# lammps/lammps-plugins

Hardware: AMD Instinct MI355X
Metric: Matom-steps/sec (higher is better)
Workload: dtype f64; 1 GPU; REBO-MoS bulk: in.rebomos-bulk cell replicated 24x24x24; atoms=3981312, style=rebomos, parallelism=spatial-dd1, transport=none (one GPU), rccl_library_is_test_double=False, thermo_every=10, displacement_check=every step, deferred on-device flag, dangerous_builds=0, inner_skin=adaptive from 1.0, late_style_list_builds_rank0=0, row_prunings_late_rank0=0, rccl_ranks=1

## Files before the change

include/mdpair_hip.h:

```cpp
#ifndef MDPAIR_HIP_H
#define MDPAIR_HIP_H

#include <stddef.h>
#include <stdint.h>

#ifdef __cplusplus
extern "C" {
#endif

#define MDP_ABI_VERSION 3

enum {
  MDP_OK = 0,
  MDP_EINVAL = -1,
  MDP_EHIP = -2,
  MDP_ENOMEM = -3,
  MDP_EOVERFLOW = -4,
  MDP_ENOTIMPL = -5,
  MDP_ESTATE = -6
};

#define MDP_EFLAG_GLOBAL 1
#define MDP_EFLAG_ATOM 2
#define MDP_VFLAG_GLOBAL 1
// ... 85 lines not shown
} mdp_md_config;

int mdp_md_setup(mdp_ctx *ctx, const mdp_md_config *cfg, const double *x, const double *v, const int *type,
                 const int *tag, const double *mass, const int *map, const int *ghost_owner,
                 const double *ghost_shift, const int *ghost_type, const int *ghost_tag);
int mdp_md_build_neighbors(mdp_ctx *ctx);
int mdp_md_initial_integrate(mdp_ctx *ctx);
int mdp_md_final_integrate(mdp_ctx *ctx);
int mdp_md_final_initial_integrate(mdp_ctx *ctx);
int mdp_md_defer_final(mdp_ctx *ctx);
int mdp_md_compute(mdp_ctx *ctx, int eflag, int vflag);
int mdp_md_compute_begin(mdp_ctx *ctx, int eflag, int vflag);
int mdp_md_compute_end(mdp_ctx *ctx, int eflag, int vflag);
int mdp_md_pack_x(mdp_ctx *ctx, int n, const int *d_sendlist, const double *d_shift, double *d_buf);
int mdp_md_unpack_x(mdp_ctx *ctx, int first_ghost, int n, const double *d_buf);
int mdp_md_pack_scalar(mdp_ctx *ctx, int which, int n, const int *d_sendlist, double *d_buf);
int mdp_md_unpack_scalar(mdp_ctx *ctx, int which, int first_ghost, int n, const double *d_buf);
int mdp_md_pack_ghost_f(mdp_ctx *ctx, int first_ghost, int n, double *d_buf);
int mdp_md_unpack_add_f(mdp_ctx *ctx, int n, const int *d_sendlist, const double *d_buf);
int mdp_md_fold_self_ghost_f(mdp_ctx *ctx);
int mdp_md_aeam_density(mdp_ctx *ctx, int eflag);
int mdp_md_aeam_force_begin(mdp_ctx *ctx, int eflag, int vflag);
int mdp_md_aeam_force(mdp_ctx *ctx, int eflag, int vflag);
int mdp_md_aeam_state(mdp_ctx *ctx, int out[4]);
int mdp_md_thermo(mdp_ctx *ctx, double out[9]);
int mdp_md_download(mdp_ctx *ctx, double *x, double *v, double *f, double *eatom);
int mdp_md_upload_x(mdp_ctx *ctx, const double *x);
int mdp_md_download_x_all(mdp_ctx *ctx, double *x_all);
void *mdp_md_ptr(mdp_ctx *ctx, const char *name);
int mdp_md_neighbor_stats(mdp_ctx *ctx, long long out[8]);
int mdp_md_prune_stats(mdp_ctx *ctx, long long out[4]);
int mdp_md_list_state(mdp_ctx *ctx, double out[8]);
int mdp_rebomos_list_info(mdp_ctx *ctx, long long out[8]);
int mdp_md_class_stats(mdp_ctx *ctx, long long out[32]);

typedef struct {
  double boxlo[3];
  double h[6];
  int procgrid[3];
  int rank;
  double cutghost;
  int self_remote;
  int nonperiodic[3];
} mdp_dd_config;

int mdp_dd_setup(mdp_ctx *ctx, const mdp_dd_config *cfg);
int mdp_dd_reneighbor(mdp_ctx *ctx);
int mdp_dd_migrate_begin(mdp_ctx *ctx, int *send_counts );
int mdp_dd_migrate_pack(mdp_ctx *ctx, double *d_buf);
int mdp_dd_migrate_end(mdp_ctx *ctx, int narrive, const double *d_buf);
int mdp_dd_borders_begin(mdp_ctx *ctx, int *send_counts );
int mdp_dd_borders_pack(mdp_ctx *ctx, double *d_buf);
int mdp_dd_borders_end(mdp_ctx *ctx, const int *recv_counts , const double *d_buf);
int mdp_dd_info(mdp_ctx *ctx, long long out[8], int *send_counts, int *recv_counts);
int mdp_dd_forward_pack(mdp_ctx *ctx, double *d_buf);
int mdp_dd_forward_unpack(mdp_ctx *ctx, const double *d_buf);
int mdp_dd_forward_scalar_pack(mdp_ctx *ctx, double *d_buf);
int mdp_dd_forward_scalar_unpack(mdp_ctx *ctx, const double *d_buf);
int mdp_dd_reverse_pack(mdp_ctx *ctx, double *d_buf);
int mdp_dd_reverse_unpack(mdp_ctx *ctx, const double *d_buf);
int mdp_dd_comm_unique_id(void *id128);
int mdp_dd_comm_library(char *buf, int cap);
int mdp_dd_comm_init(mdp_ctx *ctx, const void *id128);
int mdp_dd_comm_destroy(mdp_ctx *ctx);
int mdp_dd_comm_reneighbor(mdp_ctx *ctx);
int mdp_dd_comm_forward_begin(mdp_ctx *ctx);
// ... 94 lines not shown
```

lammps-plugins_amd/csrc/md.hip:

```cpp
#include "mdp_common.h"

#include <rocprim/rocprim.hpp>

#include <cmath>
#include <type_traits>

void mdp_rebomos_fill_dev(mdp_ctx *c, double skin);

namespace {

struct CutTables {
  double owned[MDP_AEAM_MAXT * MDP_AEAM_MAXT];
  double ghost[MDP_AEAM_MAXT * MDP_AEAM_MAXT];
  const double *g_owned;
  int ne;
  int min_type;
};

using Grid = MdpGrid;

__device__ __forceinline__ int cell_index(const Grid &g, const double4 &x, int &cx, int &cy, int &cz)
{
  cx = (int) ((x.x - g.lo[0]) * g.inv[0]);
  cy = (int) ((x.y - g.lo[1]) * g.inv[1]);
// ... 1538 lines not shown
  CutTables ct;
  memset(&ct, 0, sizeof ct);
  double maxcut = 0.0;
  MDP_TRY(aeam_cut_table(c, ct, skin, maxcut));
  return host_list_compare(c, ct, maxcut, host_total, "aeam");
}

void *mdp_md_ptr(mdp_ctx *c, const char *name)
{
  if (!c || !name) return nullptr;
  if (!strcmp(name, "x")) return c->xq.p;
  if (!strcmp(name, "v")) return c->v.p;
  if (!strcmp(name, "f")) return c->f.p;
  if (!strcmp(name, "fp")) return c->fp.p;
  if (!strcmp(name, "eatom")) return c->eatom.p;
  return nullptr;
}

int mdp_rebomos_list_info(mdp_ctx *c, long long out[8])
{
  if (!c || !out) return MDP_EINVAL;
  if (!c->rebo_packed) return mdp_fail(c, MDP_ESTATE, "rebomos lists not built yet");
  out[0] = c->lj_tiled ? 1 : 0;
  out[1] = c->ntile;
  out[2] = c->tile_cap;
  out[3] = c->tile_maxu;
  out[4] = c->lj_total;
  out[5] = c->nclus;
  out[6] = (c->lj_class_base[2] - c->lj_class_base[1]) + (c->lj_class_base[4] - c->lj_class_base[3]);
  out[7] = c->style_builds;
  return MDP_OK;
}

int mdp_md_class_stats(mdp_ctx *c, long long out[32])
{
  if (!c || !out) return MDP_EINVAL;
  for (int k = 0; k < 32; k++) out[k] = 0;
  out[30] = c->tile_maxu;
  if (c->cfg.style == 2 || (c->have_aeam && !c->have_rebomos)) {
    out[0] = c->h_ang_count;
    out[1] = c->ntile;
    out[2] = c->aeam_split;
    return MDP_OK;
  }
  for (int k = 0; k < MDP_NCLASS; k++) out[k] = c->h_class_count[k];
  for (int k = 0; k < 4; k++) out[20 + k] = c->lj_class_base[k + 1] - c->lj_class_base[k];
  if (c->lj_tiled && !c->lj_ordered) out[20] = c->ntile;
  if (c->h_pinned) {
    const int *h = mdp_pin(c, kPinOvf) + 4 * c->ovf_par;
    for (int k = 0; k < 4; k++) out[25 + k] = h[k];
    out[24] = *mdp_pin(c, kPinGeneral);
  }
  out[29] = c->tile_small;
  return MDP_OK;
}

int mdp_md_neighbor_stats(mdp_ctx *c, long long out[8])
{
  if (!c || !out) return MDP_EINVAL;
  for (int k = 0; k < 8; k++) out[k] = 0;
  out[0] = c->nb_owned_total;
  out[1] = c->nb_total - c->nb_owned_total;
  out[2] = c->lj_total;
  out[3] = c->cand_total;
  out[4] = 0;
  for (int k = 0; k < MDP_NCLASS; k++) out[4] += c->h_class_count[k];
// ... 110 lines not shown
```

lammps-plugins_amd/csrc/mdp_api.hip:

```cpp
#include "mdp_common.h"

#include <rocprim/rocprim.hpp>

#include <condition_variable>
#include <functional>
#include <mutex>
#include <thread>
#include <unistd.h>

#include <cmath>

void mdp_rebomos_fill_dev(mdp_ctx *c, double skin);

int mdp_fail(mdp_ctx *c, int code, const char *fmt, ...)
{
  char buf[1024];
  va_list ap;
  va_start(ap, fmt);
  vsnprintf(buf, sizeof buf, fmt, ap);
  va_end(ap);
  if (c) c->err = buf;
  return code;
}

// ... 731 lines not shown
  c->vatom.release();
  c->acc.release();
  c->flags.release();
  c->nb_off.release();
  c->nb.release();
  c->cand_cnt.release();
  c->cand_off.release();
  c->cand.release();
  c->lj_off.release();
  c->lj_cnt.release();
  c->lj_split.release();
  c->cl_flag.release();
  c->cl_pos.release();
  c->cl_order.release();
  c->lj.release();
  c->tu.release();
  c->tmask.release();
  c->lj16_in.release();
  c->lj_len_in.release();
  c->lj_split_in.release();
  c->cand_stage.release();
  c->lj_fixtab.release();
  c->lj_fix_stamp.release();
  c->xhold_prune.release();
  c->tile_nu.release();
  c->tile_flag.release();
  c->lj16.release();
  c->is_center.release();
  c->class_list.release();
  c->class_merged.release();
  c->class_count.release();
  c->pk_cand.release();
  c->amask.release();
  c->xhold_all.release();
  c->ovf.release();
  c->rev.release();
  c->rev16.release();
  c->host_perm.release();
  c->host_tagmap.release();
  c->host_inv.release();
  c->host_tag_dev.release();
  c->host_img.release();
  c->host_stage.release();
  host_unregister_all(c);
  for (int k = 0; k < MDP_DOWN_CHUNKS; k++)
    if (c->ev_down[k]) {
      (void) hipEventDestroy(c->ev_down[k]);
      c->ev_down[k] = nullptr;
    }
  for (int k = 0; k < MDP_UP_RING; k++) {
    if (c->h_up[k]) (void) hipHostFree(c->h_up[k]);
    if (c->ev_up[k]) (void) hipEventDestroy(c->ev_up[k]);
    c->h_up[k] = nullptr;
    c->ev_up[k] = nullptr;
  }
  if (c->h_down) (void) hipHostFree(c->h_down);
  c->h_down = nullptr;
  c->fnbr.release();
  c->fown.release();
  c->vslot.release();
  c->scan_tmp.release();
  c->rho.release();
  c->fp.release();
  c->ang_list.release();
  c->ang_count.release();
  c->v.release();
// ... 470 lines not shown
```

lammps-plugins_amd/csrc/mdp_common.h:

```cpp
#pragma once

#include <hip/hip_runtime.h>

#include <atomic>
#include <cstdarg>
#include <cstdio>
#include <cstdlib>
#include <cstring>
#include <string>
#include <utility>
#include <vector>

#include "mdpair_hip.h"

#define MDP_NEIGHMASK 0x1FFFFFFF
#define MDP_CLUSTER 2
static_assert(MDP_CLUSTER == 1 || MDP_CLUSTER == 2, "the Lennard-Jones kernels are instantiated for 1- and 2-atom clusters only");
#define MDP_ACC_SLOTS 512
#define MDP_ACC_STRIDE 16
#define MDP_NOVF_LISTS 7
#define MDP_NCLASS 20
#define MDP_NCLASS_HALF 10

inline std::atomic<long long> &mdp_device_bytes_counter()
// ... 504 lines not shown
  DevBuf<unsigned short> lj16;
  DevBuf<int> is_center;
  bool hn_on = false;
  double hn_dt = 0.0, hn_dtf = 0.0, hn_ftm2v = 0.0;
  double hn_mass[16] = {};
  DevBuf<double> hn_mass_dev;
  bool hn_v_current = false;
  int ovf_par = 0;
  bool hn_deferred_check = false;
  int ang_list_n = -1;
  bool f_prezeroed = false;
  bool f_zero_remote_due = false;
  bool aeam_img_fp = false;
  DevBuf<int> lj_fix_stamp;
  int lj_stamp = 0;
  DevBuf<unsigned short> lj_cq;
  DevBuf<int> lj_cq_cnt;
  int lj_cq_cap = 0, lj_cq_tiles = 0;
  bool lj_queue_now = false;
  DevBuf<double> lj_fixtab;
  DevBuf<int> cand_stage;
  DevBuf<int> class_list;
  DevBuf<int> class_count;
  DevBuf<int> pk_cand;
  size_t pk_base[MDP_NCLASS] = {};
  DevBuf<int> class_merged;
  size_t merged_base[MDP_NCLASS_HALF] = {};
  int h_class_count[MDP_NCLASS] = {};
  DevBuf<unsigned long long> amask;
  DevBuf<int> rev;
  DevBuf<int> rev16;
  DevBuf<int> ovf;
  int ovf_stride = 0;
  int ovf3_hot[4] = {0, 0, 0, 0};
  DevBuf<mdp_hold_t> xhold_all;
  double skin_inner = 0.0;
  double skin_inner_auto = 1.0;
  double skin_inner_cap = 1.0e9;
  long long computes_since_build = 0;
  bool stale_rebuild = false;
  long long style_builds = 0;
  long long dangerous_builds = 0;
  int sflag_set = 0;
  bool sflag_armed = false;
  bool sflag_committed[2] = {false, false};
  MdpStyleCheck sflag_chk;
  MdpStyleCheckMeta sflag_meta[2];
  hipEvent_t ev_sflag[2] = {nullptr, nullptr};
  MdpNhc nhc;
  MdpLangevin lgv;
  MdpFire fire;
  DevBuf<int> mask;
  bool mask_set = false;
  int mask_n = 0;
  int group_bit = 0, lgv_bit = 0;
  DevBuf<int> image;
  bool image_set = false;
  MdpMsd msd;
  MdpRdf rdf;
  bool final_pending = false;
  bool final_deferred_seen = false;
  bool acc_prezeroed = false;
  bool check_now = false;
  DevBuf<double> fnbr;
  DevBuf<double> fown;
  DevBuf<double> vslot;
// ... 158 lines not shown
```

lammps-plugins_amd/csrc/rebomos.hip:

```cpp
#include "mdp_common.h"

#include <type_traits>

namespace {

#ifndef MDP_LJ_WAVES
#define MDP_LJ_WAVES 4
#endif
constexpr double kPi = 3.14159265358979323846;
constexpr double kTol = 1.0e-9;

__device__ __forceinline__ void wave_lds_fence()
{
  __builtin_amdgcn_fence(__ATOMIC_RELEASE, "wavefront");
  __builtin_amdgcn_wave_barrier();
  __builtin_amdgcn_fence(__ATOMIC_ACQUIRE, "wavefront");
}

template <int G> __device__ __forceinline__ double group_sum_any(double v, const int s, const int lane);

__device__ __forceinline__ int xcd_contiguous(const int b, const int n)
{
  const int q = n >> 3, r = n & 7, xcd = b & 7, idx = b >> 3;
  return xcd * q + (xcd < r ? xcd : r) + idx;
}

template <int G> __device__ __forceinline__ double group_sum_any(double v, const int s, const int lane)
{
  if constexpr ((G & (G - 1)) == 0) {
    return group_sum<G>(v);
  } else {
    static_assert(G <= 16, "tree below starts at offset 8");
#pragma unroll
    for (int o = 8; o > 0; o >>= 1) {
      const double t = __shfl_down(v, o, 64);
// ... 18 lines not shown
  double y = __builtin_amdgcn_rcp(x);
  double e = fma(-x, y, 1.0);
  y = fma(y, e, y);
  e = fma(-x, y, 1.0);
  return fma(y, e, y);
}

__device__ __forceinline__ double rsqrt_nr(double x)
{
  double y = __builtin_amdgcn_rsq(x);
  double e = fma(-x * y, y, 1.0);
  y = fma(0.5 * y, e, y);
  e = fma(-x * y, y, 1.0);
  return fma(0.5 * y, e, y);
}

__device__ __forceinline__ double sp_switch(double r, double rmin, double rinv, double &dw)
{
  const double t = (r - rmin) * rinv;
  if (t <= 0.0) {
    dw = 0.0;
    return 1.0;
  }
  if (t >= 1.0) {
    dw = 0.0;
    return 0.0;
  }
  double s, c;
  sincospi(t, &s, &c);
  dw = -0.5 * kPi * s * rinv;
  return 0.5 * (1.0 + c);
}

__device__ __forceinline__ void sincospi_half(const double u, double &sn, double &cs)
{
  const bool fold = u > 0.25;
  const double v = fold ? 0.5 - u : u;
  const double w = v * v;
  constexpr double S[8] = {3.14159265358979312e+00, -5.16771278004996937e+00, 2.55016403987734508e+00, -5.99264529320791883e-01, 8.21458866111281910e-02, -7.37043094571434784e-03, 4.66302805767612337e-04, -2.19153534478302037e-05};
  constexpr double C[9] = {1.00000000000000000e+00, -4.93480220054467900e+00, 4.05871212641676760e+00, -1.33526276885458928e+00, 2.35330630358893123e-01, -2.58068913900140508e-02, 1.92957430940392206e-03, -1.04638104924845650e-04, 4.30306958703294391e-06};
  double ps = S[7], pc = C[8];
#pragma unroll
  for (int k = 6; k >= 0; k--) ps = fma(ps, w, S[k]);
#pragma unroll
  for (int k = 7; k >= 0; k--) pc = fma(pc, w, C[k]);
  ps *= v;
  sn = fold ? pc : ps;
  cs = fold ? ps : pc;
}

__device__ __forceinline__ double poly6(const double *c, double x, double &d)
{
  double g = c[6] * x, dg = 6.0 * c[6] * x;
  g += c[5];
  dg += 5.0 * c[5];
  g *= x;
  dg *= x;
  g += c[4];
  dg += 4.0 * c[4];
  g *= x;
  dg *= x;
  g += c[3];
  dg += 3.0 * c[3];
  g *= x;
  dg *= x;
  g += c[2];
  dg += 2.0 * c[2];
  g *= x;
  dg *= x;
  g += c[1];
  dg += c[1];
  g *= x;
  g += c[0];
  d = dg;
  return g;
}

__device__ __forceinline__ double poly6v(const double *c, double x)
{
  return (((((c[6] * x + c[5]) * x + c[4]) * x + c[3]) * x + c[2]) * x + c[1]) * x + c[0];
}

__device__ __forceinline__ double gspline_val(const double *cb, const double *cg, double c)
{
  const double gcos = poly6v(cb, c);
  if (c < 0.5) return gcos;
  const double gamma = poly6v(cg, c);
  const double psi = 0.5 * (1.0 - cospi(2.0 * (c - 0.5)));
  return gcos + psi * (gamma - gcos);
}

__device__ __forceinline__ double gspline(const double *cb, const double *cg, double c, double &dgdc)
{
  if (c < 0.5) {
    return poly6(cb, c, dgdc);
  }
  double dgcos, dgamma;
  const double gcos = poly6(cb, c, dgcos);
  const double gamma = poly6(cg, c, dgamma);
  double s, co;
  sincospi_half(c - 0.5, s, co);
  const double psi = s * s;
  const double dpsi = 2.0 * kPi * s * co;
  dgdc = dgcos + dpsi * (gamma - gcos) + psi * (dgamma - dgcos);
  return gcos + psi * (gamma - gcos);
}

constexpr int kRec = 10;
constexpr int kRecF = 9, kInvF = 7;

struct CentreOut {
  double e_acc, v0, v1, v2, v3, v4, v5;
};

__device__ __forceinline__ void finish_slot(const RebomosDev &P, const int tc, const int je_m, const int off,
                                            const double dp, const bool owned, const int eflag, const double mx,
                                            const double my, const double mz, const double mr, const double mw,
                                            const double mdw, const double mp, const double mrinv, const double mVA,
                                            double &fx, double &fy, double &fz, const double acc1, const double Csum,
                                            double *__restrict__ fnbr, double &eh, CentreOut &o)
{
  const int tm = ((unsigned) je_m) >> 30;
  const int pt = tc * 2 + tm;
  const double ux = mx * mrinv, uy = my * mrinv, uz = mz * mrinv;
  double radial = (acc1 + Csum * dp) * mdw;
  double ehalf = 0.0;
  if (mw > kTol) {
    const double ex = exp(-P.alpha[pt] * mr);
    const double pre = mw * P.A[pt] * ex;
    const double VR = pre * (1.0 + P.Q[pt] * mrinv);
    double dVR = pre * (-P.alpha[pt] - P.Q[pt] * mrinv * mrinv - P.Q[pt] * P.alpha[pt] * mrinv);
    const double swl = fast_rcp(mw) * mdw;
    dVR += VR * swl;
    double dVA = -P.beta[pt] * mVA;
    dVA += mVA * swl;
    radial += 0.5 * (dVR + mp * dVA);
    ehalf = 0.5 * (VR + mp * mVA);
  }
// ... 49 lines not shown
  const double rsq = dx * dx + dy * dy + dz * dz;
  const int tj = (int) xj.w;
  const double rc2 = P.rcmaxsq[tc * 2 + tj];
  const bool pred = valid && rsq < rc2;
  if (valid && !pred && rsq < rc2 * (1.0 + 1.0e-14)) {
    slot4[t] = make_double4(0.0, 0.0, 0.0, 0.0);
    if (vslot)
      for (int k = 0; k < 6; k++) vslot[6 * (size_t) t + k] = 0.0;
  }
  const unsigned long long bal = __ballot(pred);
  const unsigned long long gb = (bal >> glane0) & gmask;
  const int pos = n + __popcll(gb & ((1ull << s) - 1ull));
  if (pred && pos < CAP) {
    const int pt = tc * 2 + tj;
    const double rinv = rsqrt_nr(rsq);
    const double r = rsq * rinv;
    double dw;
    const double w = sp_switch(r, P.rcmin[pt], P.rcinv[pt], dw);
    double *q = rec + pos * REC;
    q[0] = dx;
    q[1] = dy;
    q[2] = dz;
    q[3] = r;
    q[4] = w;
    q[5] = dw;
    q[REC == kRec ? 8 : kInvF] = rinv;
    je[pos] = t | (tj << 30);
    nsum += w;
  }
  n += __popcll(gb);
  if (base < 64) active |= gb << base;
}

template <int G> struct CentreCfg {
  static constexpr int CAP = G;
  static constexpr int GPW = 64 / G;
  static constexpr int WPB = G == 12 ? 3 : 4;
  static constexpr int STRIDE = CAP * kRecF + 2;
  static constexpr int MSTRIDE = 2 * (G / 2) * G + 2;
  static constexpr int UA = G >= 32 ? 1 : (G >= 12 ? 2 : 4);
};


template <int G, bool LIST = false>
__global__ __launch_bounds__(64 * CentreCfg<G>::WPB) void rebo_centre_kernel(
    const RebomosDev P, const int *__restrict__ centres, const int ncent_arg, const int nlocal,
    const double4 *__restrict__ xq, const int *__restrict__ cand_off, const int *__restrict__ cand,
    const int *__restrict__ pk, unsigned long long *__restrict__ amask, double *__restrict__ fnbr,
    double *__restrict__ fown, double *__restrict__ acc, int *__restrict__ ovf, const int eflag, const int vflag,
    const int tc )
{
  using C = CentreCfg<G>;
  __shared__ double s_rec[C::WPB * C::GPW * C::STRIDE];
  __shared__ double s_mat[C::WPB * C::GPW * C::MSTRIDE];
  __shared__ int s_je[C::WPB * C::GPW * C::CAP];

  const int tid = threadIdx.x;
  const int lane = tid & 63;
  const int s = lane % G;
  const int glane0 = lane - s;
  const int gw = lane / G;
  const bool lane_ok = gw < C::GPW;
  const int grp_in_block = (tid >> 6) * C::GPW + (lane_ok ? gw : C::GPW - 1);
  const long long gid = (long long) (LIST ? (int) blockIdx.x : xcd_contiguous(blockIdx.x, gridDim.x)) * (C::WPB * C::GPW) + grp_in_block;
  const int ncent = LIST ? centres[-1] : ncent_arg;
  const bool have = lane_ok && gid < ncent;
  if (LIST) {
    int *h_count = reinterpret_cast<int *>(const_cast<int *>(pk));
    if (blockIdx.x == 0 && tid == 0) *h_count = ncent;
    const long long covered = (long long) gridDim.x * (C::WPB * C::GPW);
    for (long long e = covered + (long long) blockIdx.x * blockDim.x + tid; e < ncent; e += (long long) gridDim.x * blockDim.x)
      ovf[1 + atomicAdd(&ovf[0], 1)] = centres[e];
  }

  double *rec = s_rec + (size_t) grp_in_block * C::STRIDE;
  double *mat = s_mat + (size_t) grp_in_block * C::MSTRIDE;
  int *je = s_je + grp_in_block * C::CAP;

  constexpr int W = C::UA * G;
  int jp[C::UA];
  if (!LIST) {
#pragma unroll
    for (int u = 0; u < C::UA; u++) jp[u] = have ? pk[(size_t) gid * W + u * G + s] : -1;
// ... 17 lines not shown
  {
    double4 xj[C::UA];
#pragma unroll
    for (int u = 0; u < C::UA; u++) xj[u] = xq[jp[u] >= 0 ? jp[u] : c];
#pragma unroll
    for (int u = 0; u < C::UA; u++)
      centre_take<G, C::CAP, kRecF>(P, tc, xc, jp[u] >= 0, u * G + s, xj[u], s, glane0, u * G, rec, je, n, active, nsum,
                                    reinterpret_cast<double4 *>(fnbr) + off, nullptr);
  }
  const int ncw = wave_max_int(nc);
  for (int base = W; base < ncw; base += W) {
    int jj[C::UA];
    double4 xj[C::UA];
#pragma unroll
    for (int u = 0; u < C::UA; u++) {
      const int t = base + u * G + s;
      jj[u] = t < nc ? cand[off + t] : c;
    }
#pragma unroll
    for (int u = 0; u < C::UA; u++) xj[u] = xq[jj[u]];
#pragma unroll
    for (int u = 0; u < C::UA; u++) {
      const int t = base + u * G + s;
      centre_take<G, C::CAP, kRecF>(P, tc, xc, t < nc, t, xj[u], s, glane0, base + u * G, rec, je, n, active, nsum,
                                    reinterpret_cast<double4 *>(fnbr) + off, nullptr);
    }
  }
  if (have && s == 0) amask[c] = active;
  const bool outgrown = n > C::CAP;
  if (outgrown) {
    if (s == 0) ovf[1 + atomicAdd(&ovf[0], 1)] = c;
    n = 0;
  }
  const double Ntot = group_sum_any<G>(nsum, s, lane);
  wave_lds_fence();

  double cb[7], cg[7];
#pragma unroll
  for (int k = 0; k < 7; k++) {
    cb[k] = P.b[tc][k];
    cg[k] = P.bg[tc][k];
  }
  const double ea = exp(-P.a[tc][2] * Ntot);
  const double dp = -P.a[tc][0] + P.a[tc][1] * P.a[tc][2] * ea;
  const double PS = -P.a[tc][0] * (Ntot - 1.0) - P.a[tc][1] * ea + P.a[tc][3];

  const int nw = wave_max_int(n);
  CentreOut o = {0, 0, 0, 0, 0, 0, 0};
  const bool owned = have && c < nlocal;

  const int m = s;
  const bool act = m < n;
  double mx = 0, my = 0, mz = 0, mr = 1, mw = 0, mdw = 0, mri = 1;
  if (act) {
    const double *q = rec + m * kRecF;
    mx = q[0];
    my = q[1];
    mz = q[2];
    mr = q[3];
    mw = q[4];
    mdw = q[5];
    mri = q[kInvF];
  }
  const double ux = mx * mri, uy = my * mri, uz = mz * mri;
  const int lane_base = (threadIdx.x & 63) - s;
  double S = 0.0;
  for (int d = 1; d <= nw / 2; d++) {
    const bool mine = act && (2 * d < n || (2 * d == n && m < d));
    double give = 0.0;
    if (mine) {
      int qi = m + d;
      qi = qi >= n ? qi - n : qi;
      const double *q = rec + qi * kRecF;
      double cs = (ux * q[0] + uy * q[1] + uz * q[2]) * q[kInvF];
      cs = fmin(cs, 1.0);
      cs = fmax(cs, -1.0);
      double dg, g;
      if (__any(cs >= 0.5)) g = gspline(cb, cg, cs, dg);
      else g = poly6(cb, cs, dg);
      double *e = mat + 2 * ((d - 1) * G + m);
      e[0] = g;
      e[1] = dg;
      S += q[4] * g;
      give = mw * g;
    }
    int src = m - d;
    src = src < 0 ? src + n : src;
    const double got = __shfl(give, lane_base + (act ? src : m), 64);
    S += act ? got : 0.0;
  }
  double mC = 0.0, mp = 0.0, mVA = 0.0;
  if (act) {
    const int pt = tc * 2 + (((unsigned) je[m]) >> 30);
    mp = rsqrt_nr(1.0 + S + PS);
    mVA = -mw * P.B[pt] * exp(-P.beta[pt] * mr);
    mC = (mw > kTol) ? 0.5 * mVA * (-0.5 * mp * mp * mp) : 0.0;
    rec[m * kRecF + 6] = mC;
  }
  const double Csum = group_sum_any<G>(mC, s, lane);
  wave_lds_fence();
  double fx = 0, fy = 0, fz = 0, acc1 = 0;
  for (int d = 1; d <= nw / 2; d++) {
    const bool mine = act && (2 * d < n || (2 * d == n && m < d));
    double sx = 0, sy = 0, sz = 0, sa = 0;
    if (mine) {
      int qi = m + d;
      qi = qi >= n ? qi - n : qi;
      const double *q = rec + qi * kRecF;
      const double qrinv = q[kInvF];
      const double qx = q[0] * qrinv, qy = q[1] * qrinv, qz = q[2] * qrinv;
      double cs = ux * qx + uy * qy + uz * qz;
      cs = fmin(cs, 1.0);
      cs = fmax(cs, -1.0);
      const double *e = mat + 2 * ((d - 1) * G + m);
      const double g = e[0], dg = e[1];
      const double common = (mC * q[4] + q[6] * mw) * dg;
      const double cm = common * mri, cq = common * qrinv;
      fx += cm * (qx - cs * ux);
      fy += cm * (qy - cs * uy);
      fz += cm * (qz - cs * uz);
      acc1 += q[6] * g;
      sx = cq * (ux - cs * qx);
      sy = cq * (uy - cs * qy);
      sz = cq * (uz - cs * qz);
      sa = mC * g;
    }
    int src = m - d;
    src = src < 0 ? src + n : src;
    const int from = lane_base + (act ? src : m);
    const double rx = __shfl(sx, from, 64), ry = __shfl(sy, from, 64), rz = __shfl(sz, from, 64);
    const double ra = __shfl(sa, from, 64);
    if (act) {
      fx += rx;
      fy += ry;
      fz += rz;
      acc1 += ra;
    }
  }
  double eh = 0.0;
  if (act)
    finish_slot(P, tc, je[m], off, dp, owned, eflag, mx, my, mz, mr, mw, mdw, mp, mri, mVA, fx, fy, fz, acc1, Csum,
                fnbr, eh, o);
  const double ox = group_sum_any<G>(act ? fx : 0.0, s, lane), oy = group_sum_any<G>(act ? fy : 0.0, s, lane), oz = group_sum_any<G>(act ? fz : 0.0, s, lane);
  const double oe = (eflag & MDP_EFLAG_ATOM) ? group_sum_any<G>(eh, s, lane) : 0.0;
  if (owned && s == 0 && !outgrown) reinterpret_cast<double4 *>(fown)[c] = make_double4(-ox, -oy, -oz, oe);
  centre_tally(o, acc, eflag, vflag);
}

constexpr int kC3Block = 256;
__global__ __launch_bounds__(kC3Block) void rebo_centre3_kernel(
    const RebomosDev P, const int *__restrict__ centres, const int ncent, const int nlocal,
    const double4 *__restrict__ xq, const int *__restrict__ cand_off, const int *__restrict__ cand,
    const int *__restrict__ pk, unsigned long long *__restrict__ amask, double *__restrict__ fnbr,
    double *__restrict__ fown, double *__restrict__ acc, int *__restrict__ ovf3 ,
    int *__restrict__ ovf_general , const int eflag, const int vflag, const int tc)
{
  constexpr int W = CentreCfg<4>::UA * 4;
  static_assert(W == 16, "four int4 per centre");
  const long long gid = (long long) xcd_contiguous(blockIdx.x, gridDim.x) * kC3Block + threadIdx.x;
  const bool have = gid < ncent;
  int jp[W];
  {
    const int4 *__restrict__ p4 = reinterpret_cast<const int4 *>(pk) + (have ? gid : 0) * (W / 4);
#pragma unroll
    for (int q = 0; q < W / 4; q++) {
      const int4 v = p4[q];
      jp[4 * q] = have ? v.x : -1;
      jp[4 * q + 1] = have ? v.y : -1;
      jp[4 * q + 2] = have ? v.z : -1;
      jp[4 * q + 3] = have ? v.w : -1;
    }
  }
  int c = 0, off = 0, nc = 0;
  double4 xc = make_double4(0, 0, 0, 0);
  if (have) {
    c = centres[gid];
    off = cand_off[c];
    nc = cand_off[c + 1] - off;
// ... 2897 lines not shown
  if (c->md || !c->have_rebomos || c->have_aeam || !c->rebo_packed || !c->nall) return MDP_OK;
  MDP_TRY(rebomos_check_launch(c, 0.5 * c->skin_inner));
  c->host_check_armed = true;
  return MDP_OK;
}

static int rebomos_lists_stale(mdp_ctx *c, bool &stale)
{
  stale = false;
  if (!c->nall) return MDP_OK;
  int *h = mdp_pin(c, kPinHostCheck);
  if (!c->md && c->host_check_armed) {
    c->host_check_armed = false;
    stale = h[0] != 0;
    if (c->prune_valid && h[2]) c->prune_stale = true;
    return MDP_OK;
  }
  const bool deferred_host = !c->md && c->hn_on && c->hn_deferred_check && !c->check_now;
  if ((!c->md && !deferred_host) || c->check_now) {
    mdp_sflag_drop(c);
    c->check_now = false;
    MDP_TRY(rebomos_check_launch(c, 0.5 * c->skin_inner));
    MDP_HIP(c, hipStreamSynchronize(c->stream));
    stale = h[0] != 0;
    if (c->prune_valid && h[2]) c->prune_stale = true;
    return MDP_OK;
  }
  bool toofar = false;
  MDP_TRY(mdp_sflag_collect(c, &stale, &toofar));
  if (toofar) c->dangerous_builds++;
  return MDP_OK;
}

template <int G>
static void launch_centre(mdp_ctx *c, int kg, int eflag, int vflag, int part)
{
  for (int elem = 0; elem < 2; elem++) {
    const int k = 2 * kg + elem + (part == 1 ? MDP_NCLASS_HALF : 0);
    const int n = c->h_class_count[k] + (part == 2 ? c->h_class_count[k + MDP_NCLASS_HALF] : 0);
    if (n <= 0) continue;
    const int *list = part == 2 ? c->class_merged.p + c->merged_base[k] : c->class_list.p + (size_t) k * c->nall;
    constexpr int per_block = CentreCfg<G>::WPB * CentreCfg<G>::GPW;
    const int grid = (n + per_block - 1) / per_block;
    rebo_centre_kernel<G><<<grid, 64 * CentreCfg<G>::WPB, 0, c->stream>>>(c->rebomos, list, n, c->nlocal,
                                                       c->xq.p, c->cand_off.p, c->cand.p, c->pk_cand.p + c->pk_base[k],
                                                       c->amask.p, c->fnbr.p, c->fown.p, c->acc.p, c->ovf.p, eflag, vflag,
                                                       elem);
  }
}

static void launch_centre3(mdp_ctx *c, int eflag, int vflag, int part)
{
  for (int elem = 0; elem < 2; elem++) {
    const int k = elem + (part == 1 ? MDP_NCLASS_HALF : 0);
    const int n = c->h_class_count[k] + (part == 2 ? c->h_class_count[k + MDP_NCLASS_HALF] : 0);
    if (n <= 0) continue;
    const int *clist = part == 2 ? c->class_merged.p + c->merged_base[k] : c->class_list.p + (size_t) k * c->nall;
    const int q = (part == 1 ? 2 : 0) + elem;
    int *list = c->ovf.p + (size_t) (q + 1) * c->ovf_stride + 1;
    int *h_cnt = mdp_pin(c, kPinOvf) + 4 * c->ovf_par + q;
    if (*h_cnt > 0) c->ovf3_hot[q] = 64;
    else if (c->ovf3_hot[q] > 0) c->ovf3_hot[q]--;
    const bool list_mode = c->ovf3_hot[q] > 0;
    rebo_centre3_kernel<<<(n + kC3Block - 1) / kC3Block, kC3Block, 0, c->stream>>>(c->rebomos, clist, n,
                                                                c->nlocal, c->xq.p, c->cand_off.p, c->cand.p,
                                                                c->pk_cand.p + c->pk_base[k], c->amask.p, c->fnbr.p,
                                                                c->fown.p, c->acc.p, list, list_mode ? nullptr : c->ovf.p,
                                                                eflag, vflag, elem);
    if (!list_mode) continue;
    constexpr int per_block = CentreCfg<8>::WPB * CentreCfg<8>::GPW;
    long long est = 4 * (long long) *h_cnt + 2 * per_block;
    if (est > n) est = n;
    const int grid = (int) ((est + per_block - 1) / per_block);
    rebo_centre_kernel<8, true><<<grid, 64 * CentreCfg<8>::WPB, 0, c->stream>>>(
        c->rebomos, list, 0, c->nlocal, c->xq.p, c->cand_off.p, c->cand.p, h_cnt, c->amask.p, c->fnbr.p, c->fown.p,
        c->acc.p, c->ovf.p, eflag, vflag, elem);
  }
}

int mdp_tile_prune(mdp_ctx *c, const double lim_rsq[4])
{
  hipStream_t st = c->stream;
  const int nrow = c->ntile * MDP_TILE;
  MDP_HIP(c, c->lj_len_in.reserve(nrow + 1));
  MDP_HIP(c, c->lj_split_in.reserve(nrow + 1));
  MDP_HIP(c, c->xhold_prune.reserve((size_t) 3 * c->nall + 3));
  if (c->prune_copied_epoch != c->prune_epoch) {
    MDP_HIP(c, c->lj16_in.reserve((size_t) c->lj_total + 256));
    MDP_HIP(c, hipMemcpyAsync(c->lj16_in.p + c->lj_total, c->lj16.p + c->lj_total, sizeof(unsigned short) * 256,
                              hipMemcpyDeviceToDevice, st));
    c->prune_copied_epoch = c->prune_epoch;
  }
  PruneLimits lim;
  for (int k = 0; k < 4; k++) lim.rsq[k] = lim_rsq[k];
  const int capL = (c->tile_maxu + 1 + 1) & ~1;
  const size_t lds = (size_t) capL * 3 * sizeof(double) + (size_t) 2 * c->tile_rowmax + 32;
  if (c->tile_rowmax <= 0 || lds > 160 * 1024) {
    c->prune_valid = false;
    return MDP_OK;
  }
#define MDP_TP(CLV)                                                                                                    \
  do {                                                                                                                 \
    if (lds > 48 * 1024)                                                                                               \
      MDP_HIP(c, hipFuncSetAttribute((const void *) tile_prune_kernel<CLV>, hipFuncAttributeMaxDynamicSharedMemorySize, \
                                     (int) lds));                                                                      \
    tile_prune_kernel<CLV><<<c->ntile, 256, lds, st>>>(lim, c->nlocal, c->nclus, c->xq.p, c->tile_cap, capL, c->tu.p,    \
                                                       c->tile_nu.p, c->lj_off.p, c->lj_split.p, c->lj16.p,            \
                                                       c->lj16_in.p, c->lj_len_in.p, c->lj_split_in.p);               \
  } while (0)
// ... 172 lines not shown
    MDP_HIP(c, hipGetLastError());
  }
  const int capL = (c->tile_maxu + 1 + 7) & ~7;
  const size_t lds = (size_t) capL * 3 * sizeof(double);
  int *h_count = mdp_pin(c, queue ? kPinCubicWalk : kPinCubic);
  long long want = (long long) *h_count + *h_count / 4 + 256;
  const int grid = (int) (want < c->ntile ? want : c->ntile);
  const int *fix_list = c->ovf.p + (size_t) (queue ? 6 : 5) * c->ovf_stride;
#define MDP_LJC(CLV, EVV)                                                                                            \
  do {                                                                                                                \
    if (lds > 48 * 1024)                                                                                              \
      MDP_HIP(c, hipFuncSetAttribute((const void *) rebo_lj_cubic_kernel<CLV, EVV>,                                   \
                                     hipFuncAttributeMaxDynamicSharedMemorySize, (int) lds));                         \
    rebo_lj_cubic_kernel<CLV, EVV><<<grid, 256, lds, c->stream>>>(                                                    \
        c->lj_fixtab.p, fix_list, c->nlocal, c->nclus, c->xq.p, c->tile_cap, c->tu.p, c->tile_nu.p, c->lj_off.p,      \
        pruned ? c->lj_len_in.p : nullptr, pruned ? c->lj_split_in.p : c->lj_split.p,                                 \
        pruned ? c->lj16_in.p : c->lj16.p, c->f.p, c->eatom.p, c->acc.p, eflag, vflag, h_count);                      \
  } while (0)
  const bool ev = eflag || vflag;
  if (c->cluster == 1) {
    if (ev) MDP_LJC(1, true);
    else MDP_LJC(1, false);
  } else {
    if (ev) MDP_LJC(2, true);
    else MDP_LJC(2, false);
  }
#undef MDP_LJC
  MDP_HIP(c, hipGetLastError());
  return MDP_OK;
}

static int launch_centres(mdp_ctx *c, int eflag, int vflag, int parts, int which = 3, bool first = true)
{
  if ((parts & 1) && first) c->ovf_par ^= 1;
  hipStream_t st = c->stream;
  if (c->centre_split && parts == 3 && which == 3) {
    launch_centre3(c, eflag, vflag, 2);
    launch_centre<8>(c, 1, eflag, vflag, 2);
    launch_centre<12>(c, 2, eflag, vflag, 2);
    launch_centre<16>(c, 3, eflag, vflag, 2);
    launch_centre<32>(c, 4, eflag, vflag, 2);
  } else
    for (int part = 0; part < 2; part++) {
      if (!((parts >> part) & 1)) continue;
      const int w = part == 0 ? which : 3;
      if (w & 1) launch_centre3(c, eflag, vflag, part);
      if (w & 2) {
        launch_centre<8>(c, 1, eflag, vflag, part);
        launch_centre<12>(c, 2, eflag, vflag, part);
        launch_centre<16>(c, 3, eflag, vflag, part);
        launch_centre<32>(c, 4, eflag, vflag, part);
      }
    }
  MDP_HIP(c, hipGetLastError());
  if (!(parts & 2)) return MDP_OK;
  int total = 0;
  for (int k = 0; k < MDP_NCLASS; k++) total += c->h_class_count[k];
  const int grid = total > 0 ? (total / 8 + 1 < 64 ? total / 8 + 1 : 64) : 0;
  mdp_time_mark(c, 1);
  if (grid)
    rebo_centre_general_kernel<false><<<grid, 256, 0, st>>>(c->rebomos, c->ovf.p, -1, c->nlocal, c->xq.p,
                                                            c->cand_off.p, c->cand.p, c->amask.p, c->fnbr.p,
                                                            c->fown.p, nullptr, nullptr, c->acc.p, c->flags.p,
                                                            eflag, vflag, mdp_pin(c, kPinOvf) + 4 * c->ovf_par,
                                                            c->ovf_stride, mdp_pin(c, kPinGeneral));
  MDP_HIP(c, hipGetLastError());
// ... 114 lines not shown
```

lammps-plugins_amd/host/capi.py:

```python
from __future__ import annotations

import ctypes as C
import os

import numpy as np

PKG_DIR = os.path.dirname(os.path.dirname(os.path.abspath(__file__)))
LIB_PATH = os.path.join(PKG_DIR, "libmdpair_hip.so")

D22 = (C.c_double * 2) * 2


class RebomosParams(C.Structure):
    _fields_ = [(n, D22) for n in ("rcmin", "rcmax", "rcmaxsq", "Q", "alpha", "A", "BIJc", "Beta")] + [
        ("b", (C.c_double * 2) * 7), ("bg", (C.c_double * 2) * 7), ("a", (C.c_double * 2) * 4)] + [
        (n, D22) for n in ("rcLJmin", "rcLJmax", "epsilon", "sigma", "lj1", "lj2", "lj3", "lj4")]


class AeamTables(C.Structure):
    _fields_ = [("ntypes", C.c_int), ("nelements", C.c_int), ("nnonangular", C.c_int),
                ("nrhomax", C.c_int), ("nrmax", C.c_int), ("nfrho", C.c_int), ("nrhor", C.c_int), ("nz2r", C.c_int),
                ("nrho", C.POINTER(C.c_int)), ("drho", C.POINTER(C.c_double)),
                ("nr", C.POINTER(C.c_int)), ("dr", C.POINTER(C.c_double)), ("cut", C.POINTER(C.c_double)),
                ("type2frho", C.POINTER(C.c_int)), ("type2rhor", C.POINTER(C.c_int)), ("type2z2r", C.POINTER(C.c_int)),
# ... 36 lines not shown
FIRE_DEFAULTS = dict(dmax=0.1, tmax=10.0, tmin=0.02, delaystep=20, dtgrow=1.1, dtshrink=0.5, alpha0=0.25,
                     alphashrink=0.99, halfstepback=True, initialdelay=True)
BOLTZ_METAL = 8.617343e-5


STYLE_REBOMOS, STYLE_AEAM = 1, 2
EXPORTS = [
    "mdp_abi_version", "mdp_device_count", "mdp_create", "mdp_destroy", "mdp_last_error", "mdp_set_stream",
    "mdp_sync", "mdp_rebomos_set_params", "mdp_rebomos_read_file", "mdp_rebomos_params_from_scalars",
    "mdp_aeam_set_tables", "mdp_aeam_file_read", "mdp_aeam_file_info", "mdp_aeam_file_build", "mdp_aeam_file_free", "mdp_set_atoms_host", "mdp_set_positions_host",
    "mdp_set_box_host", "mdp_host_ghosts_derived",
    "mdp_set_neighbors_host", "mdp_set_skin", "mdp_set_neighbors_csr_host", "mdp_rebomos_compute_host", "mdp_aeam_density_host",
    "mdp_aeam_force_host", "mdp_md_setup", "mdp_md_build_neighbors", "mdp_md_initial_integrate",
    "mdp_md_final_integrate", "mdp_md_final_initial_integrate", "mdp_md_compute", "mdp_md_compute_begin", "mdp_md_compute_end", "mdp_md_pack_x", "mdp_md_unpack_x", "mdp_md_pack_scalar",
    "mdp_md_unpack_scalar", "mdp_md_pack_ghost_f", "mdp_md_unpack_add_f", "mdp_md_fold_self_ghost_f",
    "mdp_md_aeam_density", "mdp_md_aeam_force", "mdp_md_thermo", "mdp_md_download", "mdp_md_upload_x", "mdp_md_ptr",
    "mdp_md_neighbor_stats", "mdp_md_class_stats", "mdp_md_prune_stats", "mdp_hnve_setup", "mdp_hnve_off", "mdp_hnve_upload_v",
    "mdp_hnve_initial", "mdp_hnve_final", "mdp_hnve_download", "mdp_rebomos_list_info", "mdp_set_timing", "mdp_get_timing",
    "mdp_device_bytes", "mdp_host_release", "mdp_rebomos_check_host_list",
    "mdp_dd_setup", "mdp_dd_reneighbor", "mdp_dd_migrate_begin", "mdp_dd_migrate_pack", "mdp_dd_migrate_end",
    "mdp_dd_borders_begin", "mdp_dd_borders_pack", "mdp_dd_borders_end", "mdp_dd_info", "mdp_dd_forward_pack",
    "mdp_dd_forward_unpack", "mdp_dd_forward_scalar_pack", "mdp_dd_forward_scalar_unpack", "mdp_dd_reverse_pack",
    "mdp_dd_reverse_unpack", "mdp_md_moved_async", "mdp_md_integrate_check", "mdp_md_download_int", "mdp_md_download_x_all",
    "mdp_dd_comm_unique_id", "mdp_dd_comm_library", "mdp_dd_comm_init", "mdp_dd_comm_destroy", "mdp_dd_comm_reneighbor",
    "mdp_dd_comm_forward_begin", "mdp_dd_comm_forward_end", "mdp_dd_comm_forward_scalar", "mdp_dd_comm_reverse",
    "mdp_dd_comm_allreduce", "mdp_dd_comm_step_begin", "mdp_dd_comm_step_end", "mdp_dd_comm_step_info", "mdp_aeam_device_lists", "mdp_rebomos_host_list", "mdp_aeam_check_host_list",
    "mdp_md_defer_final", "mdp_md_list_state", "mdp_md_aeam_force_begin", "mdp_md_aeam_state", "mdp_dd_comm_aeam_exchange_begin", "mdp_dd_comm_aeam_exchange_end",
    "mdp_nhc_setup", "mdp_nhc_run", "mdp_nhc_state", "mdp_nhc_set_state", "mdp_nhc_off",
    "mdp_langevin_setup", "mdp_langevin_run", "mdp_langevin_tally", "mdp_langevin_off",
    "mdp_fire_setup", "mdp_fire_iterate", "mdp_fire_state", "mdp_fire_off",
    "mdp_md_set_mask", "mdp_hnve_set_mask", "mdp_integrate_group", "mdp_langevin_group",
    "mdp_md_set_image", "mdp_md_download_unwrapped", "mdp_msd_setup", "mdp_msd_sums", "mdp_msd_info", "mdp_msd_off",
    "mdp_rdf_setup", "mdp_rdf_counts", "mdp_rdf_info", "mdp_rdf_off",
]


class MdpError(RuntimeError):
    def __init__(self, code, text):
        super().__init__(f"libmdpair_hip: error {code}: {text}")
        self.code = code


_lib = None


def lib():
    global _lib
    if _lib is None:
        if not os.path.exists(LIB_PATH):
            raise FileNotFoundError(f"{LIB_PATH} not built: run `python __graft_entry__.py` (make -C lammps-plugins_amd)")
        try:
            import torch
        except ImportError:
            pass
        _lib = C.CDLL(os.environ.get("MDP_LIB_PATH") or LIB_PATH)
        _lib.mdp_last_error.restype = C.c_char_p
        _lib.mdp_md_ptr.restype = C.c_void_p
        _lib.mdp_device_bytes.restype = C.c_double
    return _lib


def _dp(a):
    return None if a is None else a.ctypes.data_as(C.POINTER(C.c_double))


def _ip(a):
# ... 282 lines not shown
        out = (C.c_double * 9)()
        self._ck(self.L.mdp_md_thermo(self.h, out))
        o = list(out)
        return dict(ke=o[0], pe=o[1], virial=np.array(o[2:8]), maxdisp2=o[8])

    def md_download(self, nlocal, want=("x", "v", "f")):
        arrs = {k: (np.zeros((nlocal, 3)) if k in want else None) for k in ("x", "v", "f")}
        ea = np.zeros(nlocal) if "eatom" in want else None
        self._ck(self.L.mdp_md_download(self.h, _dp(arrs["x"]), _dp(arrs["v"]), _dp(arrs["f"]), _dp(ea)))
        arrs["eatom"] = ea
        return arrs

    def md_download_x_all(self, nall):
        x = np.zeros((max(nall, 1), 3))
        self._ck(self.L.mdp_md_download_x_all(self.h, _dp(x)))
        return x[:nall]

    def md_upload_x(self, x):
        x = np.ascontiguousarray(x, dtype=np.float64)
        self._ck(self.L.mdp_md_upload_x(self.h, _dp(x)))

    def md_ptr(self, name: str) -> int:
        p = self.L.mdp_md_ptr(self.h, name.encode())
        if not p:
            raise MdpError(-1, f"mdp_md_ptr({name}) returned NULL")
        return int(p)

    def rebomos_list_info(self):
        out = (C.c_longlong * 8)()
        self._ck(self.L.mdp_rebomos_list_info(self.h, out))
        keys = ("tiled", "tiles", "union_stride", "union_max", "row_entries", "clusters", "large_tiles", "builds")
        return dict(zip(keys, (int(v) for v in out)))

    def md_neighbor_stats(self):
        out = (C.c_longlong * 8)()
        self._ck(self.L.mdp_md_neighbor_stats(self.h, out))
        return list(out)

    def hnve_setup(self, dt, ftm2v, mass_per_type):
        m = np.ascontiguousarray(mass_per_type, dtype=np.float64)
        self._ck(self.L.mdp_hnve_setup(self.h, C.c_double(dt), C.c_double(ftm2v), _dp(m), C.c_int(len(m) - 1)))

    def hnve_off(self):
        self._ck(self.L.mdp_hnve_off(self.h))

    def hnve_upload_v(self, v):
        v = np.ascontiguousarray(v, dtype=np.float64)
        self._ck(self.L.mdp_hnve_upload_v(self.h, _dp(v)))

    def hnve_initial(self):
        m, d = C.c_int(0), C.c_int(0)
        self._ck(self.L.mdp_hnve_initial(self.h, C.byref(m), C.byref(d)))
        return bool(m.value), bool(d.value)

    def hnve_final(self):
        self._ck(self.L.mdp_hnve_final(self.h))

    def hnve_download(self, nlocal, want=("x", "v", "f")):
        out = {k: np.zeros((nlocal, 3)) for k in want}
        self._ck(self.L.mdp_hnve_download(self.h, _dp(out.get("x")), _dp(out.get("v")), _dp(out.get("f"))))
        return out

    def nhc_setup(self, t_start, t_stop, t_period, nf, tchain=3, tloop=1, drag=0.0, boltz=BOLTZ_METAL, mvv2e=1.0364269e-4):
        cfg = NhcConfig(t_start, t_stop, t_period, tchain, tloop, drag, nf, boltz, mvv2e)
        self._ck(self.L.mdp_nhc_setup(self.h, C.byref(cfg)))

# ... 310 lines not shown
```

Baseline: 1441 Matom-steps/s.

## Add full-group fast path for REBO-MoS centre bond-angle loops

Adds a specialised path in the rebo_centre_kernel for waves where every group holds exactly G neighbours (G<=16). It unrolls the pairwise angle loops at compile time, exchanges partner contributions via ds_bpermute instead of the generic loop, and loads the sin/cos series coefficients from constant memory with the leading terms pinned in registers. The aim is to cut loop control, divergence and register/literal pressure in the angle and force loops. Waves with any group not full fall back to the old loop, and an optional env-controlled atomic counter records which path each wave took.

```diff
diff --git a/include/mdpair_hip.h b/include/mdpair_hip.h
--- a/include/mdpair_hip.h
+++ b/include/mdpair_hip.h
@@ -141,6 +141,7 @@
 int mdp_md_prune_stats(mdp_ctx *ctx, long long out[4]);
 int mdp_md_list_state(mdp_ctx *ctx, double out[8]);
 int mdp_rebomos_list_info(mdp_ctx *ctx, long long out[8]);
+int mdp_rebomos_centre_paths(mdp_ctx *ctx, long long out[2], int reset);
 int mdp_md_class_stats(mdp_ctx *ctx, long long out[32]);
 
 typedef struct {
diff --git a/lammps-plugins_amd/csrc/md.hip b/lammps-plugins_amd/csrc/md.hip
--- a/lammps-plugins_amd/csrc/md.hip
+++ b/lammps-plugins_amd/csrc/md.hip
@@ -1594,6 +1594,19 @@
   return MDP_OK;
 }
 
+int mdp_rebomos_centre_paths(mdp_ctx *c, long long out[2], int reset)
+{
+  if (!c || !out) return MDP_EINVAL;
+  out[0] = out[1] = 0;
+  if (!c->centre_paths.p) return MDP_OK;
+  unsigned long long h[2];
+  MDP_TRY(mdp_read_one(c, c->centre_paths.p, sizeof h, h));
+  out[0] = (long long) h[0];
+  out[1] = (long long) h[1];
+  if (reset) MDP_HIP(c, hipMemsetAsync(c->centre_paths.p, 0, sizeof h, c->stream));
+  return MDP_OK;
+}
+
 int mdp_md_class_stats(mdp_ctx *c, long long out[32])
 {
   if (!c || !out) return MDP_EINVAL;
diff --git a/lammps-plugins_amd/csrc/mdp_api.hip b/lammps-plugins_amd/csrc/mdp_api.hip
--- a/lammps-plugins_amd/csrc/mdp_api.hip
+++ b/lammps-plugins_amd/csrc/mdp_api.hip
@@ -787,6 +787,7 @@
   c->class_count.release();
   c->pk_cand.release();
   c->amask.release();
+  c->centre_paths.release();
   c->xhold_all.release();
   c->ovf.release();
   c->rev.release();
diff --git a/lammps-plugins_amd/csrc/mdp_common.h b/lammps-plugins_amd/csrc/mdp_common.h
--- a/lammps-plugins_amd/csrc/mdp_common.h
+++ b/lammps-plugins_amd/csrc/mdp_common.h
@@ -560,6 +560,9 @@
   DevBuf<int> rev16;
   DevBuf<int> ovf;
   int ovf_stride = 0;
+  DevBuf<unsigned long long> centre_paths;
+  bool centre_full_now = true;
+  unsigned long long *centre_cnt_now = nullptr;
   int ovf3_hot[4] = {0, 0, 0, 0};
   DevBuf<mdp_hold_t> xhold_all;
   double skin_inner = 0.0;
diff --git a/lammps-plugins_amd/csrc/rebomos.hip b/lammps-plugins_amd/csrc/rebomos.hip
--- a/lammps-plugins_amd/csrc/rebomos.hip
+++ b/lammps-plugins_amd/csrc/rebomos.hip
@@ -1,6 +1,11 @@
 #include "mdp_common.h"
 
 #include <type_traits>
+
+#define MDP_SINPI_COEFFS 3.14159265358979312e+00, -5.16771278004996937e+00, 2.55016403987734508e+00, -5.99264529320791883e-01, 8.21458866111281910e-02, -7.37043094571434784e-03, 4.66302805767612337e-04, -2.19153534478302037e-05
+#define MDP_COSPI_COEFFS 1.00000000000000000e+00, -4.93480220054467900e+00, 4.05871212641676760e+00, -1.33526276885458928e+00, 2.35330630358893123e-01, -2.58068913900140508e-02, 1.92957430940392206e-03, -1.04638104924845650e-04, 4.30306958703294391e-06
+__constant__ double mdp_sinpi_series[8] = {MDP_SINPI_COEFFS};
+__constant__ double mdp_cospi_series[9] = {MDP_COSPI_COEFFS};
 
 namespace {
 
@@ -85,18 +90,45 @@
   return 0.5 * (1.0 + c);
 }
 
-__device__ __forceinline__ void sincospi_half(const double u, double &sn, double &cs)
+struct SeriesLead {
+  double s7, c8;
+};
+__device__ __forceinline__ SeriesLead series_lead()
+{
+  SeriesLead l = {mdp_sinpi_series[7], mdp_cospi_series[8]};
+  asm("" : "+v"(l.s7));
+  asm("" : "+v"(l.c8));
+  return l;
+}
+
+struct SeriesLiteral {};
+
+template <class L>
+__device__ __forceinline__ void sincospi_half(const double u, double &sn, double &cs, const L &lead)
 {
   const bool fold = u > 0.25;
   const double v = fold ? 0.5 - u : u;
   const double w = v * v;
-  constexpr double S[8] = {3.14159265358979312e+00, -5.16771278004996937e+00, 2.55016403987734508e+00, -5.99264529320791883e-01, 8.21458866111281910e-02, -7.37043094571434784e-03, 4.66302805767612337e-04, -2.19153534478302037e-05};
-  constexpr double C[9] = {1.00000000000000000e+00, -4.93480220054467900e+00, 4.05871212641676760e+00, -1.33526276885458928e+00, 2.35330630358893123e-01, -2.58068913900140508e-02, 1.92957430940392206e-03, -1.04638104924845650e-04, 4.30306958703294391e-06};
-  double ps = S[7], pc = C[8];
-#pragma unroll
-  for (int k = 6; k >= 0; k--) ps = fma(ps, w, S[k]);
-#pragma unroll
-  for (int k = 7; k >= 0; k--) pc = fma(pc, w, C[k]);
+  double ps, pc;
+  if constexpr (std::is_same<L, SeriesLead>::value) {
+    const double *S = mdp_sinpi_series, *C = mdp_cospi_series;
+    ps = lead.s7;
+    pc = lead.c8;
+#pragma unroll
+    for (int k = 6; k >= 0; k--) ps = fma(ps, w, S[k]);
+#pragma unroll
+    for (int k = 7; k >= 1; k--) pc = fma(pc, w, C[k]);
+    pc = fma(pc, w, 1.0);
+  } else {
+    constexpr double S[8] = {MDP_SINPI_COEFFS};
+    constexpr double C[9] = {MDP_COSPI_COEFFS};
+    ps = S[7];
+    pc = C[8];
+#pragma unroll
+    for (int k = 6; k >= 0; k--) ps = fma(ps, w, S[k]);
+#pragma unroll
+    for (int k = 7; k >= 0; k--) pc = fma(pc, w, C[k]);
+  }
   ps *= v;
   sn = fold ? pc : ps;
   cs = fold ? ps : pc;
@@ -143,7 +175,8 @@
   return gcos + psi * (gamma - gcos);
 }
 
-__device__ __forceinline__ double gspline(const double *cb, const double *cg, double c, double &dgdc)
+template <class L>
+__device__ __forceinline__ double gspline(const double *cb, const double *cg, double c, double &dgdc, const L &lead)
 {
   if (c < 0.5) {
     return poly6(cb, c, dgdc);
@@ -152,11 +185,16 @@
   const double gcos = poly6(cb, c, dgcos);
   const double gamma = poly6(cg, c, dgamma);
   double s, co;
-  sincospi_half(c - 0.5, s, co);
+  sincospi_half(c - 0.5, s, co, lead);
   const double psi = s * s;
   const double dpsi = 2.0 * kPi * s * co;
   dgdc = dgcos + dpsi * (gamma - gcos) + psi * (dgamma - dgcos);
   return gcos + psi * (gamma - gcos);
+}
+
+__device__ __forceinline__ double gspline(const double *cb, const double *cg, double c, double &dgdc)
+{
+  return gspline(cb, cg, c, dgdc, SeriesLiteral{});
 }
 
 constexpr int kRec = 10;
@@ -272,6 +310,20 @@
   if (base < 64) active |= gb << base;
 }
 
+__device__ __forceinline__ double bpermute_f64(const int addr4, const double v)
+{
+  const int lo = __builtin_amdgcn_ds_bpermute(addr4, __double2loint(v));
+  const int hi = __builtin_amdgcn_ds_bpermute(addr4, __double2hiint(v));
+  return __hiloint2double(hi, lo);
+}
+
+template <int K> __device__ __forceinline__ double unread_f64()
+{
+  double v;
+  asm("; unread value %1" : "=v"(v) : "n"(K));
+  return v;
+}
+
 template <int G> struct CentreCfg {
   static constexpr int CAP = G;
   static constexpr int GPW = 64 / G;
@@ -288,7 +340,9 @@
     const double4 *__restrict__ xq, const int *__restrict__ cand_off, const int *__restrict__ cand,
     const int *__restrict__ pk, unsigned long long *__restrict__ amask, double *__restrict__ fnbr,
     double *__restrict__ fown, double *__restrict__ acc, int *__restrict__ ovf, const int eflag, const int vflag,
-    const int tc )
+    const int tc ,
+    const int full_on ,
+    unsigned long long *__restrict__ path_cnt )
 {
   using C = CentreCfg<G>;
   __shared__ double s_rec[C::WPB * C::GPW * C::STRIDE];
@@ -372,6 +426,8 @@
     if (s == 0) ovf[1 + atomicAdd(&ovf[0], 1)] = c;
     n = 0;
   }
+  int c_own = (have && c < nlocal && !outgrown) ? c : -1;
+  asm("" : "+v"(c_own));
   const double Ntot = group_sum_any<G>(nsum, s, lane);
   wave_lds_fence();
 
@@ -385,9 +441,9 @@
   const double dp = -P.a[tc][0] + P.a[tc][1] * P.a[tc][2] * ea;
   const double PS = -P.a[tc][0] * (Ntot - 1.0) - P.a[tc][1] * ea + P.a[tc][3];
 
+  const SeriesLead lead = series_lead();
   const int nw = wave_max_int(n);
   CentreOut o = {0, 0, 0, 0, 0, 0, 0};
-  const bool owned = have && c < nlocal;
 
   const int m = s;
   const bool act = m < n;
@@ -404,7 +460,48 @@
   }
   const double ux = mx * mri, uy = my * mri, uz = mz * mri;
   const int lane_base = (threadIdx.x & 63) - s;
+  constexpr bool kFullPath = G <= 16;
+  constexpr bool kAllLanes = C::GPW * G == 64;
+  const int lane_again = (int) __builtin_amdgcn_mbcnt_hi(~0u, __builtin_amdgcn_mbcnt_lo(~0u, 0u));
+  bool full = false;
+  if constexpr (kFullPath) full = full_on && __all(!lane_ok || n == G);
+  if (path_cnt && __any(have) && lane == 0) atomicAdd(&path_cnt[full ? 0 : 1], 1ull);
+  const double *qm = rec + m * kRecF;
+  const double *qwrap = qm - G * kRecF;
+  double *em = mat + 2 * m;
+  int from4[kFullPath ? G / 2 : 1];
+  if constexpr (kFullPath)
+    if (full) {
+#pragma unroll
+      for (int d = 1; d <= G / 2; d++) from4[d - 1] = 4 * (lane - d + (m < d ? G : 0));
+    }
   double S = 0.0;
+  if (full) {
+    if constexpr (kFullPath)
+      if (kAllLanes || lane_again < C::GPW * G) {
+#pragma unroll
+        for (int d = 1; d <= G / 2; d++) {
+          const bool half = 2 * d == G;
+          const double *q = (m >= G - d ? qwrap : qm) + d * kRecF;
+          double give = unread_f64<0>();
+          if (!half || m < d) {
+            double cs = (ux * q[0] + uy * q[1] + uz * q[2]) * q[kInvF];
+            cs = fmin(cs, 1.0);
+            cs = fmax(cs, -1.0);
+            double dg, g;
+            if (__any(cs >= 0.5)) g = gspline(cb, cg, cs, dg, lead);
+            else g = poly6(cb, cs, dg);
+            em[2 * (d - 1) * G] = g;
+            em[2 * (d - 1) * G + 1] = dg;
+            S += q[4] * g;
+            give = mw * g;
+          }
+          const double got = bpermute_f64(from4[d - 1], give);
+          if (!half || m >= d) S += got;
+          __builtin_amdgcn_sched_barrier(0);
+        }
+      }
+  } else
   for (int d = 1; d <= nw / 2; d++) {
     const bool mine = act && (2 * d < n || (2 * d == n && m < d));
     double give = 0.0;
@@ -416,7 +513,7 @@
       cs = fmin(cs, 1.0);
       cs = fmax(cs, -1.0);
       double dg, g;
-      if (__any(cs >= 0.5)) g = gspline(cb, cg, cs, dg);
+      if (__any(cs >= 0.5)) g = gspline(cb, cg, cs, dg, lead);
       else g = poly6(cb, cs, dg);
       double *e = mat + 2 * ((d - 1) * G + m);
       e[0] = g;
@@ -440,6 +537,45 @@
   const double Csum = group_sum_any<G>(mC, s, lane);
   wave_lds_fence();
   double fx = 0, fy = 0, fz = 0, acc1 = 0;
+  if (full) {
+    if constexpr (kFullPath)
+      if (kAllLanes || lane_again < C::GPW * G) {
+#pragma unroll
+        for (int d = 1; d <= G / 2; d++) {
+          const bool half = 2 * d == G;
+          const double *q = (m >= G - d ? qwrap : qm) + d * kRecF;
+          double sx = unread_f64<0>(), sy = unread_f64<1>(), sz = unread_f64<2>(), sa = unread_f64<3>();
+          if (!half || m < d) {
+            const double qrinv = q[kInvF];
+            const double qx = q[0] * qrinv, qy = q[1] * qrinv, qz = q[2] * qrinv;
+            double cs = ux * qx + uy * qy + uz * qz;
+            cs = fmin(cs, 1.0);
+            cs = fmax(cs, -1.0);
+            const double g = em[2 * (d - 1) * G], dg = em[2 * (d - 1) * G + 1];
+            const double common = (mC * q[4] + q[6] * mw) * dg;
+            const double cm = common * mri, cq = common * qrinv;
+            fx += cm * (qx - cs * ux);
+            fy += cm * (qy - cs * uy);
+            fz += cm * (qz - cs * uz);
+            acc1 += q[6] * g;
+            sx = cq * (ux - cs * qx);
+            sy = cq * (uy - cs * qy);
+            sz = cq * (uz - cs * qz);
+            sa = mC * g;
+          }
+          const int from = from4[d - 1];
+          const double rx = bpermute_f64(from, sx), ry = bpermute_f64(from, sy), rz = bpermute_f64(from, sz);
+          const double ra = bpermute_f64(from, sa);
+          if (!half || m >= d) {
+            fx += rx;
+            fy += ry;
+            fz += rz;
+            acc1 += ra;
+          }
+          __builtin_amdgcn_sched_barrier(0);
+        }
+      }
+  } else
   for (int d = 1; d <= nw / 2; d++) {
     const bool mine = act && (2 * d < n || (2 * d == n && m < d));
     double sx = 0, sy = 0, sz = 0, sa = 0;
@@ -479,11 +615,11 @@
   }
   double eh = 0.0;
   if (act)
-    finish_slot(P, tc, je[m], off, dp, owned, eflag, mx, my, mz, mr, mw, mdw, mp, mri, mVA, fx, fy, fz, acc1, Csum,
+    finish_slot(P, tc, je[m], off, dp, c_own >= 0, eflag, mx, my, mz, mr, mw, mdw, mp, mri, mVA, fx, fy, fz, acc1, Csum,
                 fnbr, eh, o);
   const double ox = group_sum_any<G>(act ? fx : 0.0, s, lane), oy = group_sum_any<G>(act ? fy : 0.0, s, lane), oz = group_sum_any<G>(act ? fz : 0.0, s, lane);
   const double oe = (eflag & MDP_EFLAG_ATOM) ? group_sum_any<G>(eh, s, lane) : 0.0;
-  if (owned && s == 0 && !outgrown) reinterpret_cast<double4 *>(fown)[c] = make_double4(-ox, -oy, -oz, oe);
+  if (c_own >= 0 && s == 0) reinterpret_cast<double4 *>(fown)[c_own] = make_double4(-ox, -oy, -oz, oe);
   centre_tally(o, acc, eflag, vflag);
 }
 
@@ -3447,6 +3583,22 @@
   return MDP_OK;
 }
 
+static int centre_path_mode(mdp_ctx *c)
+{
+  const char *fe = getenv("MDP_CENTRE_FULL");
+  c->centre_full_now = !(fe && atoi(fe) == 0);
+  const char *ce = getenv("MDP_CENTRE_COUNT");
+  c->centre_cnt_now = nullptr;
+  if (ce && atoi(ce) != 0) {
+    if (!c->centre_paths.p) {
+      MDP_HIP(c, c->centre_paths.reserve(2));
+      MDP_HIP(c, hipMemsetAsync(c->centre_paths.p, 0, sizeof(unsigned long long) * 2, c->stream));
+    }
+    c->centre_cnt_now = c->centre_paths.p;
+  }
+  return MDP_OK;
+}
+
 template <int G>
 static void launch_centre(mdp_ctx *c, int kg, int eflag, int vflag, int part)
 {
@@ -3460,7 +3612,7 @@
     rebo_centre_kernel<G><<<grid, 64 * CentreCfg<G>::WPB, 0, c->stream>>>(c->rebomos, list, n, c->nlocal,
                                                        c->xq.p, c->cand_off.p, c->cand.p, c->pk_cand.p + c->pk_base[k],
                                                        c->amask.p, c->fnbr.p, c->fown.p, c->acc.p, c->ovf.p, eflag, vflag,
-                                                       elem);
+                                                       elem, c->centre_full_now ? 1 : 0, c->centre_cnt_now);
   }
 }
 
@@ -3489,7 +3641,7 @@
     const int grid = (int) ((est + per_block - 1) / per_block);
     rebo_centre_kernel<8, true><<<grid, 64 * CentreCfg<8>::WPB, 0, c->stream>>>(
         c->rebomos, list, 0, c->nlocal, c->xq.p, c->cand_off.p, c->cand.p, h_cnt, c->amask.p, c->fnbr.p, c->fown.p,
-        c->acc.p, c->ovf.p, eflag, vflag, elem);
+        c->acc.p, c->ovf.p, eflag, vflag, elem, c->centre_full_now ? 1 : 0, c->centre_cnt_now);
   }
 }
 
@@ -3728,6 +3880,7 @@
 
 static int launch_centres(mdp_ctx *c, int eflag, int vflag, int parts, int which = 3, bool first = true)
 {
+  if ((parts & 1) && first) MDP_TRY(centre_path_mode(c));
   if ((parts & 1) && first) c->ovf_par ^= 1;
   hipStream_t st = c->stream;
   if (c->centre_split && parts == 3 && which == 3) {
diff --git a/lammps-plugins_amd/host/capi.py b/lammps-plugins_amd/host/capi.py
--- a/lammps-plugins_amd/host/capi.py
+++ b/lammps-plugins_amd/host/capi.py
@@ -92,6 +92,7 @@
     "mdp_md_set_mask", "mdp_hnve_set_mask", "mdp_integrate_group", "mdp_langevin_group",
     "mdp_md_set_image", "mdp_md_download_unwrapped", "mdp_msd_setup", "mdp_msd_sums", "mdp_msd_info", "mdp_msd_off",
     "mdp_rdf_setup", "mdp_rdf_counts", "mdp_rdf_info", "mdp_rdf_off",
+    "mdp_rebomos_centre_paths",
 ]
 
 
@@ -440,6 +441,11 @@
         keys = ("tiled", "tiles", "union_stride", "union_max", "row_entries", "clusters", "large_tiles", "builds")
         return dict(zip(keys, (int(v) for v in out)))
 
+    def rebomos_centre_paths(self, reset=True):
+        out = (C.c_longlong * 2)()
+        self._ck(self.L.mdp_rebomos_centre_paths(self.h, out, C.c_int(1 if reset else 0)))
+        return int(out[0]), int(out[1])
+
     def md_neighbor_stats(self):
         out = (C.c_longlong * 8)()
         self._ck(self.L.mdp_md_neighbor_stats(self.h, out))
```

Result: faster. 1504 Matom-steps/s, median of 6 (+4.3%).
